# microsoft/tf-gnn-samples

Hardware: AMD Instinct MI355X
Metric: edges/sec (whole node), RGCN PPI h=256 training, distinct batches (the reference's epoch-loop definition) (higher is better)
Workload: dtype f32; 1 GPU; C2: RGCN on synthetic PPI-shaped batches (~16 graphs, ~1.88 M edges, ~32 k nodes each), 3 edge types [fwd,self,bkwd], h=256, 3 layers, sum aggregation, 1/in-de…; graphs_per_rank=64, max_nodes_in_batch=35964, input_pipeline=ResidentDataset, parallelism=dp1-by-graph

## Files before the change

include/relgnn.h:

```cpp
#ifndef RELGNN_H_
#define RELGNN_H_

#include <stddef.h>
#include <stdint.h>

#ifdef __cplusplus
extern "C" {
#endif

#define RELGNN_ABI_VERSION 1

#define RELGNN_OK 0
#define RELGNN_EINVAL 1
#define RELGNN_ENOSPC 2
#define RELGNN_EHIP 3
#define RELGNN_EUNSUPPORTED 4

#define RELGNN_ERRFLAG_INDEX_OUT_OF_RANGE 1u

#define RELGNN_AGG_SUM 0
#define RELGNN_AGG_MEAN 1
#define RELGNN_AGG_SQRT_N 2
#define RELGNN_AGG_MAX 3

// ... 273 lines not shown
                                int32_t batch, uint16_t* out, void* stream);
int relgnn_limb_split_multi_f32(int32_t n, const float* const* X, const int64_t* ldx, const int32_t* rows, const int32_t* cols,
                                const int32_t* transpose, uint16_t* const* out, const int32_t* kt_offset, const int32_t* kt_total,
                                void* stream);
int relgnn_limb_gemm_f32(int32_t act, const uint16_t* A, const uint16_t* B, const float* bias, const void* zeros, float* C,
                         int64_t ldc, int32_t M, int32_t N, int32_t K, void* stream);
int relgnn_limb_gemm_xf32(int32_t act, const float* A, int64_t lda, const uint16_t* B, const float* bias, const void* zeros,
                          float* C, int64_t ldc, int32_t M, int32_t N, int32_t K, void* stream);
int64_t relgnn_limb16_elements(int64_t rows, int64_t cols);
int relgnn_limb16_split_multi_f32(int32_t n, const float* const* X, const int64_t* ldx, const int32_t* rows, const int32_t* cols,
                                  const int32_t* transpose, uint16_t* const* out, const int32_t* kt_offset, const int32_t* kt_total,
                                  const int32_t* image, int32_t n_images, float* wmax, void* stream);
int relgnn_limb16_gemm_xf32(int32_t act, const float* A, int64_t lda, const float* xmax, int32_t xgroups, const uint16_t* B,
                            const float* wmax, const float* bias, const void* zeros, float* C, int64_t ldc, int32_t M, int32_t N,
                            int32_t K, void* stream);
int relgnn_limb16_gemm_tn_f32(const float* A, int64_t lda, const float* G, int64_t ldg, const float* amax, int32_t a_cols_per_scale,
                              const float* gmax, int32_t g_cols_per_scale, float* P, int32_t V, int32_t J, int32_t C, void* stream);
int64_t relgnn_col_absmax_workspace_bytes(int32_t rows, int32_t cols);
int relgnn_col_absmax_f32(const float* X, int64_t ldx, int32_t rows, int32_t cols, float* out, void* workspace,
                          int64_t workspace_bytes, void* stream);
int relgnn_absmax_f32(const float* x, int64_t n, float* out, void* stream);
int relgnn_limb_gemm_xf32_dact(int32_t act, const float* A, int64_t lda, const uint16_t* B, const float* bias, const void* zeros,
                               int32_t dact, const float* Y, int64_t ldy, float* C, int64_t ldc, int32_t M, int32_t N, int32_t K,
                               void* stream);
int relgnn_limb16_gemm_xf32_dact(int32_t act, const float* A, int64_t lda, const float* xmax, int32_t xgroups, const uint16_t* B,
                                 const float* wmax, const float* bias, const void* zeros, int32_t dact, const float* Y, int64_t ldy,
                                 float* C, int64_t ldc, int32_t M, int32_t N, int32_t K, void* stream);
#define RELGNN_HANDOVER_FUSED_MATRIX 1
#define RELGNN_HANDOVER_FUSED_GATHER 2
#define RELGNN_HANDOVER_PC_MATRIX 4
#define RELGNN_HANDOVER_PC_PRODUCER 8
int relgnn_limb_gemm_xf32_pc(int32_t act, const float* A, int64_t lda, const uint16_t* B, const float* bias, int32_t dact,
                             const float* Y, int64_t ldy, float* C, int64_t ldc, int32_t M, int32_t N, int32_t K, int32_t* status,
                             void* stream);
int relgnn_limb_gemm_xf32_pc_supported(int32_t act, int32_t M, int32_t N, int32_t K);
int relgnn_rgcn_fused_fwd(const float* H, int64_t num_rows_h, int64_t ldh, const int32_t* rowptr, int32_t num_nodes,
                          int32_t num_edge_types, const int32_t* col, const float* w, const uint16_t* w_limbs, const float* bias,
                          int32_t act, float* bucket_sums, int64_t lds, float* out, int64_t ldo, int32_t d_in, int32_t d_out,
                          int32_t* status, void* stream);
int relgnn_limb_dense_sel_f32(int32_t layout, int32_t act, const float* A, int64_t lda, const int32_t* a_rows, const float* B,
                              int64_t ldb, int32_t num_b, int64_t b_batch_stride, const int32_t* b_select, int32_t rows_per_select,
                              const float* bias, const void* zeros, uint16_t* limb_ws, int64_t limb_ws_elements, float* C,
                              int64_t ldc, int32_t M, int32_t N, int32_t K, void* stream);
int relgnn_limb_gemm_sel_xf32(int32_t act, const float* A, int64_t lda, const int32_t* a_rows, const uint16_t* B_limbs, int32_t num_b,
                              const int32_t* b_select, int32_t rows_per_select, const float* bias, const void* zeros, float* C,
                              int64_t ldc, int32_t M, int32_t N, int32_t K, void* stream);
int relgnn_limb_gemm_sel_pc_supported(int32_t M, int32_t N, int32_t K, int32_t rows_per_select);
int relgnn_limb_gemm_sel_pc_xf32(const float* A, int64_t lda, const int32_t* a_rows, const uint16_t* B_limbs, int32_t num_b,
                                 const int32_t* b_select, int32_t rows_per_select, const void* zeros, float* C, int64_t ldc,
                                 int32_t M, int32_t N, int32_t K, int32_t* status, void* stream);
int64_t relgnn_limb_gemm_tn_chunks(int32_t V, int32_t J, int32_t C);
int relgnn_limb_gemm_tn_f32(const float* A, int64_t lda, const float* G, int64_t ldg, float* P, int32_t V, int32_t J, int32_t C,
                            void* stream);
int relgnn_limb_gemm_tn_tiles_f32(const float* A, int64_t lda, const int32_t* a_rows, const float* G, int64_t ldg,
                                  const void* zeros, float* part, int32_t P, int32_t rows_per_tile, int32_t J, int32_t C,
                                  void* stream);
int relgnn_limb_dense_f32(int32_t layout, int32_t act, const float* A, int64_t lda, const float* B, int64_t ldb, const float* bias,
                          const void* zeros, uint16_t* limb_ws, int64_t limb_ws_elements, float* C, int64_t ldc, int32_t M,
                          int32_t N, int32_t K, void* stream);


int relgnn_rgdcn_apply_fwd(int32_t mode, int32_t weight_act, int32_t out_act, const float* A, const float* P,
                           int64_t p_node_stride, int64_t p_type_stride, int64_t p_channel_stride, int32_t num_nodes,
                           int32_t num_edge_types, int32_t num_channels, int32_t channel_dim, const int32_t* rowptr_t,
                           float* out, void* stream);
int relgnn_rgdcn_apply_bwd(int32_t weight_act, const float* A, const float* P, int64_t p_node_stride, int64_t p_type_stride,
                           int64_t p_channel_stride, int32_t num_nodes, int32_t num_edge_types, int32_t num_channels,
                           int32_t channel_dim, const float* G, float* gA, float* gP, void* stream);

#ifdef __cplusplus
}
#endif
#endif
```

tf_gnn_samples_amd/_lib.py:

```python
import ctypes
from pathlib import Path

import torch

_PKG_DIR = Path(__file__).resolve().parent
LIB_PATH = _PKG_DIR / "librelgnn.so"

OK, EINVAL, ENOSPC, EHIP, EUNSUPPORTED = 0, 1, 2, 3, 4
ERRFLAG_INDEX_OUT_OF_RANGE = 1

AGG_SUM, AGG_MEAN, AGG_SQRT_N, AGG_MAX = 0, 1, 2, 3
MT_MAX = 48
ACT_LINEAR, ACT_TANH, ACT_RELU, ACT_LEAKY_RELU, ACT_ELU, ACT_SELU, ACT_GELU = range(7)
ACT_NAMES = ("linear", "tanh", "relu", "leaky_relu", "elu", "selu", "gelu")

_c_i32, _c_i64, _c_f32 = ctypes.c_int32, ctypes.c_int64, ctypes.c_float
_ptr = ctypes.c_void_p

_SIGNATURES = {
    "relgnn_abi_version": (ctypes.c_int, []),
    "relgnn_status_string": (ctypes.c_char_p, [ctypes.c_int]),
    "relgnn_relational_keys": (ctypes.c_int, [_ptr, _c_i64, _c_i32, _c_i32, _c_i32, _c_i64, _ptr, _ptr, _ptr, _ptr]),
    "relgnn_relational_keys2": (ctypes.c_int, [_ptr, _c_i64, _c_i32, _c_i32, _c_i32, _c_i64, _ptr, _ptr, _ptr, _ptr, _ptr, _ptr]),
    "relgnn_relational_keys_all": (ctypes.c_int, [_ptr, _ptr, _c_i32, _c_i32, _ptr, _ptr, _ptr, _ptr, _ptr, _ptr]),
# ... 23 lines not shown
    "relgnn_rgat_bwd_logits": (ctypes.c_int, [_ptr, _c_i64, _c_i32, _c_i32, _ptr, _ptr, _ptr, _c_i32, _c_i32, _ptr, _c_f32, _ptr, _ptr, _ptr, _c_i64, _ptr, _ptr, _ptr]),
    "relgnn_rgat_bwd_msg": (ctypes.c_int, [_c_i32, _c_i32, _ptr, _c_i64, _ptr, _ptr, _ptr, _ptr, _ptr, _c_i64, _ptr, _c_i64, _ptr, _ptr]),
    "relgnn_rgat_alpha": (ctypes.c_int, [_ptr, _ptr, _c_i32, _ptr, _c_i32, _c_i32, _ptr, _c_f32, _ptr, _ptr]),
    "relgnn_headw_reduce": (ctypes.c_int, [_ptr, _c_i64, _c_i64, _c_i32, _c_i32, _ptr, _c_i64, _c_i32, _ptr, _ptr, _ptr, _ptr, _c_i64, _ptr, _ptr, _ptr]),
    "relgnn_rgat_dz": (ctypes.c_int, [_ptr, _c_i64, _c_i64, _c_i32, _c_i32, _ptr, _ptr, _ptr, _c_i32, _c_i32, _ptr, _c_f32, _ptr, _ptr, _ptr, _c_i64, _ptr, _ptr, _ptr]),
    "relgnn_pair_fwd": (ctypes.c_int, [_c_i32, _c_i32, _ptr, _c_i64, _ptr, _c_i64, _c_i32, _ptr, _c_i32, _c_i32, _ptr, _ptr, _ptr, _c_i64, _ptr]),
    "relgnn_pair_bwd_q": (ctypes.c_int, [_c_i32, _ptr, _c_i64, _ptr, _c_i64, _c_i32, _ptr, _c_i32, _c_i32, _ptr, _ptr, _ptr, _c_i64, _ptr, _c_i64, _ptr, _ptr]),
    "relgnn_pair_bwd_p": (ctypes.c_int, [_c_i32, _ptr, _c_i64, _ptr, _c_i64, _c_i32, _ptr, _c_i64, _ptr, _ptr, _ptr, _ptr, _c_i64, _ptr, _c_i64, _ptr]),
    "relgnn_column_sum_workspace_bytes": (ctypes.c_size_t, [_c_i64, _c_i32]),
    "relgnn_column_sum": (ctypes.c_int, [_ptr, _c_i64, _c_i32, _c_i64, _ptr, _ptr, ctypes.c_size_t, _ptr]),
    "relgnn_mt_l2norm_workspace_bytes": (ctypes.c_size_t, []),
    "relgnn_mt_l2norm": (ctypes.c_int, [_ptr, _ptr, _c_i32, _ptr, _ptr, ctypes.c_size_t, _ptr]),
    "relgnn_mt_adam_clip": (ctypes.c_int, [_ptr, _ptr, _ptr, _ptr, _ptr, _c_i32, _ptr, _c_f32, _c_f32, _c_f32, _c_f32, _c_f32, _ptr]),
    "relgnn_adam_step_size": (ctypes.c_int, [_ptr, _c_f32, _c_f32, _c_f32, _ptr]),
    "relgnn_mt_adam_clip_devlr": (ctypes.c_int, [_ptr, _ptr, _ptr, _ptr, _ptr, _c_i32, _ptr, _c_f32, _ptr, _c_f32, _c_f32, _c_f32, _ptr]),
    "relgnn_sigmoid_ce_stats_workspace_bytes": (ctypes.c_size_t, []),
    "relgnn_sigmoid_ce_stats": (ctypes.c_int, [_ptr, _ptr, _c_i64, _c_f32, _ptr, _ptr, ctypes.c_size_t, _ptr]),
    "relgnn_sigmoid_ce_bwd": (ctypes.c_int, [_ptr, _ptr, _c_i64, _ptr, _c_f32, _ptr, _ptr, _ptr]),
    "relgnn_sigmoid_ce_bwd_padded": (ctypes.c_int, [_ptr, _ptr, _c_i64, _c_i32, _ptr, _c_f32, _ptr, _ptr, _c_i32, _ptr]),
    "relgnn_gru_gates_fwd": (ctypes.c_int, [_ptr, _ptr, _ptr, _c_i64, _c_i32, _ptr, _ptr, _ptr, _ptr]),
    "relgnn_gru_cell_fwd_supported": (ctypes.c_int, [_c_i32, _c_i32, _c_i32]),
    "relgnn_gru_cell_fwd_xf32": (ctypes.c_int, [_ptr, _c_i64, _ptr, _c_i64, _ptr, _ptr, _ptr, _c_i32, _ptr, _ptr, _ptr, _ptr, _ptr,
                                                _c_i64, _c_i32, _c_i32, _ptr, _ptr]),
    "relgnn_gru_cell_bwd_xf32": (ctypes.c_int, [_ptr, _c_i64, _ptr, _ptr, _ptr, _c_i64, _ptr, _ptr, _ptr, _c_i32, _ptr, _ptr, _ptr, _c_i64,
                                                _c_i32, _c_i32, _ptr, _ptr]),
    "relgnn_gru_out_fwd": (ctypes.c_int, [_ptr, _ptr, _ptr, _ptr, _c_i64, _c_i32, _c_i32, _ptr, _ptr, _ptr]),
    "relgnn_gru_out_bwd": (ctypes.c_int, [_ptr, _ptr, _ptr, _ptr, _c_i64, _c_i32, _c_i32, _ptr, _ptr, _ptr, _ptr, _ptr]),
    "relgnn_gru_gates_bwd": (ctypes.c_int, [_ptr, _ptr, _ptr, _ptr, _ptr, _c_i64, _c_i32, _ptr, _ptr, _ptr]),
    "relgnn_pair_materialize": (ctypes.c_int, [_c_i32, _ptr, _c_i64, _ptr, _c_i64, _c_i32, _ptr, _ptr, _c_i64, _ptr, _ptr, _c_i64, _ptr]),
    "relgnn_rgat_scores_groups": (_c_i64, [_c_i64]),
    "relgnn_rgat_scores_fwd": (ctypes.c_int, [_ptr, _c_i64, _c_i32, _c_i32, _ptr, _c_i32, _c_i64, _ptr, _ptr, _ptr]),
    "relgnn_rgat_scores_bwd": (ctypes.c_int, [_ptr, _c_i64, _c_i32, _c_i32, _ptr, _c_i32, _c_i64, _ptr, _ptr, _ptr, _c_i64, _ptr, _c_i64, _ptr]),
    "relgnn_layer_norm_groups": (_c_i64, [_c_i64, _c_i32]),
    "relgnn_layer_norm_fwd": (ctypes.c_int, [_ptr, _c_i64, _c_i64, _c_i32, _ptr, _ptr, _c_f32, _ptr, _c_i64, _ptr, _ptr, _ptr]),
    "relgnn_layer_norm_bwd": (ctypes.c_int, [_ptr, _c_i64, _ptr, _c_i64, _c_i64, _c_i32, _ptr, _ptr, _ptr, _ptr, _c_i64, _ptr, _c_i64, _ptr]),
    "relgnn_panel_gemm_zeros_floats": (ctypes.c_int, []),
    "relgnn_panel_gemm_f32": (ctypes.c_int, [_c_i32, _c_i32, _ptr, _c_i64, _ptr, _ptr, _c_i64, _ptr, _c_i32, _c_i64, _ptr, _ptr, _ptr,
                                             _c_i64, _c_i32, _c_i32, _c_i32, _c_i32, _c_i64, _c_i64, _c_i64, _c_i32, _ptr]),
    "relgnn_limb_elements": (_c_i64, [_c_i64, _c_i64]),
    "relgnn_limb_split_f32": (ctypes.c_int, [_ptr, _c_i64, _c_i32, _c_i32, _c_i32, _ptr, _ptr]),
    "relgnn_limb_gemm_f32": (ctypes.c_int, [_c_i32, _ptr, _ptr, _ptr, _ptr, _ptr, _c_i64, _c_i32, _c_i32, _c_i32, _ptr]),
    "relgnn_limb_gemm_xf32": (ctypes.c_int, [_c_i32, _ptr, _c_i64, _ptr, _ptr, _ptr, _ptr, _c_i64, _c_i32, _c_i32, _c_i32, _ptr]),
    "relgnn_limb_gemm_xf32_dact": (ctypes.c_int, [_c_i32, _ptr, _c_i64, _ptr, _ptr, _ptr, _c_i32, _ptr, _c_i64, _ptr, _c_i64, _c_i32, _c_i32,
                                                  _c_i32, _ptr]),
    "relgnn_limb16_gemm_xf32_dact": (ctypes.c_int, [_c_i32, _ptr, _c_i64, _ptr, _c_i32, _ptr, _ptr, _ptr, _ptr, _c_i32, _ptr, _c_i64, _ptr,
                                                    _c_i64, _c_i32, _c_i32, _c_i32, _ptr]),
    "relgnn_rgcn_fused_fwd": (ctypes.c_int, [_ptr, _c_i64, _c_i64, _ptr, _c_i32, _c_i32, _ptr, _ptr, _ptr, _ptr, _c_i32, _ptr, _c_i64, _ptr,
                                             _c_i64, _c_i32, _c_i32, _ptr, _ptr]),
    "relgnn_limb_gemm_xf32_pc": (ctypes.c_int, [_c_i32, _ptr, _c_i64, _ptr, _ptr, _c_i32, _ptr, _c_i64, _ptr, _c_i64, _c_i32, _c_i32, _c_i32,
                                                _ptr, _ptr]),
    "relgnn_limb_gemm_xf32_pc_supported": (ctypes.c_int, [_c_i32, _c_i32, _c_i32, _c_i32]),
    "relgnn_limb_gemm_tn_chunks": (_c_i64, [_c_i32, _c_i32, _c_i32]),
    "relgnn_limb_gemm_tn_f32": (ctypes.c_int, [_ptr, _c_i64, _ptr, _c_i64, _ptr, _c_i32, _c_i32, _c_i32, _ptr]),
    "relgnn_limb_gemm_tn_tiles_f32": (ctypes.c_int, [_ptr, _c_i64, _ptr, _ptr, _c_i64, _ptr, _ptr, _c_i32, _c_i32, _c_i32, _c_i32, _ptr]),
    "relgnn_limb16_gemm_tn_f32": (ctypes.c_int, [_ptr, _c_i64, _ptr, _c_i64, _ptr, _c_i32, _ptr, _c_i32, _ptr, _c_i32, _c_i32, _c_i32, _ptr]),
    "relgnn_col_absmax_workspace_bytes": (ctypes.c_int64, [_c_i32, _c_i32]),
    "relgnn_col_absmax_f32": (ctypes.c_int, [_ptr, _c_i64, _c_i32, _c_i32, _ptr, _ptr, _c_i64, _ptr]),
    "relgnn_absmax_f32": (ctypes.c_int, [_ptr, _c_i64, _ptr, _ptr]),
    "relgnn_limb16_elements": (_c_i64, [_c_i64, _c_i64]),
    "relgnn_limb16_split_multi_f32": (ctypes.c_int, [_c_i32, _ptr, _ptr, _ptr, _ptr, _ptr, _ptr, _ptr, _ptr, _ptr, _c_i32, _ptr, _ptr]),
    "relgnn_limb16_gemm_xf32": (ctypes.c_int, [_c_i32, _ptr, _c_i64, _ptr, _c_i32, _ptr, _ptr, _ptr, _ptr, _ptr, _c_i64, _c_i32, _c_i32,
                                               _c_i32, _ptr]),
    "relgnn_limb_split_multi_f32": (ctypes.c_int, [_c_i32, _ptr, _ptr, _ptr, _ptr, _ptr, _ptr, _ptr, _ptr, _ptr]),
    "relgnn_limb_split_batch_f32": (ctypes.c_int, [_ptr, _c_i64, _c_i64, _c_i32, _c_i32, _c_i32, _c_i32, _ptr, _ptr]),
    "relgnn_limb_dense_sel_f32": (ctypes.c_int, [_c_i32, _c_i32, _ptr, _c_i64, _ptr, _ptr, _c_i64, _c_i32, _c_i64, _ptr, _c_i32, _ptr, _ptr,
                                                 _ptr, _c_i64, _ptr, _c_i64, _c_i32, _c_i32, _c_i32, _ptr]),
    "relgnn_limb_gemm_sel_xf32": (ctypes.c_int, [_c_i32, _ptr, _c_i64, _ptr, _ptr, _c_i32, _ptr, _c_i32, _ptr, _ptr, _ptr, _c_i64, _c_i32,
                                                 _c_i32, _c_i32, _ptr]),
    "relgnn_limb_gemm_sel_pc_supported": (ctypes.c_int, [_c_i32, _c_i32, _c_i32, _c_i32]),
    "relgnn_limb_gemm_sel_pc_xf32": (ctypes.c_int, [_ptr, _c_i64, _ptr, _ptr, _c_i32, _ptr, _c_i32, _ptr, _ptr, _c_i64, _c_i32, _c_i32,
                                                    _c_i32, _ptr, _ptr]),
    "relgnn_fill_rows_f32": (ctypes.c_int, [_ptr, _c_i64, _c_i32, _ptr, _c_i64, ctypes.c_float, _ptr]),
    "relgnn_limb_dense_f32": (ctypes.c_int, [_c_i32, _c_i32, _ptr, _c_i64, _ptr, _c_i64, _ptr, _ptr, _ptr, _c_i64, _ptr, _c_i64, _c_i32,
                                             _c_i32, _c_i32, _ptr]),
    "relgnn_blaslt_gemm_f32": (ctypes.c_int, [_c_i32, _c_i32, _ptr, _c_i64, _ptr, _c_i64, _ptr, _ptr, _c_i64, _c_i32, _c_i32, _c_i32, _c_i32,
                                              _c_i64, _c_i64, _c_i64, _c_i32, _ptr, _c_i64, _ptr]),
    "relgnn_gemm_tn_stream_workspace_bytes": (_c_i64, [_c_i32, _c_i32, _c_i64]),
    "relgnn_gemm_tn_stream_f32": (ctypes.c_int, [_ptr, _c_i64, _ptr, _c_i64, _ptr, _c_i64, _c_i32, _c_i32, _c_i64, _c_i32, _ptr, _c_i64, _ptr]),
    "relgnn_gemm_tn_stream_group_workspace_bytes": (_c_i64, [_c_i32, _ptr, _ptr, _c_i64, _c_i32]),
    "relgnn_gemm_tn_stream_group_f32": (ctypes.c_int, [_c_i32, _ptr, _ptr, _ptr, _ptr, _ptr, _ptr, _ptr, _ptr, _c_i64, _ptr, _ptr, _c_i64,
                                                       _ptr]),
    "relgnn_gemm_tn_stream_blocks_f32": (ctypes.c_int, [_ptr, _c_i64, _ptr, _c_i64, _ptr, _c_i64, _c_i64, _c_i32, _c_i32, _c_i32, _c_i64,
                                                        _c_i32, _ptr, _c_i64, _ptr]),
    "relgnn_sum_slabs_tail_f32": (ctypes.c_int, [_ptr, _c_i32, _c_i32, _c_i32, _ptr, _c_i64, _ptr, _c_i64, _c_i32, _ptr, _ptr]),
    "relgnn_rgdcn_apply_fwd": (ctypes.c_int, [_c_i32, _c_i32, _c_i32, _ptr, _ptr, _c_i64, _c_i64, _c_i64, _c_i32, _c_i32, _c_i32, _c_i32, _ptr, _ptr, _ptr]),
    "relgnn_rgdcn_apply_bwd": (ctypes.c_int, [_c_i32, _ptr, _ptr, _c_i64, _c_i64, _c_i64, _c_i32, _c_i32, _c_i32, _c_i32, _ptr, _ptr, _ptr, _ptr]),
    "relgnn_batch_gather": (ctypes.c_int, [_ptr, _c_i32, _c_i32, _c_i64] + [_ptr] * 6 + [_c_i64, _c_i64, _c_i64, _c_i32, _ptr, _ptr, _ptr,
                                           _ptr, _ptr, _ptr, _ptr, _ptr, _ptr]),
    "relgnn_plan_assemble": (ctypes.c_int, [_ptr, _c_i32, _c_i32, _c_i64] + [_ptr] * 8 + [_c_i64, _c_i64] + [_ptr] * 16 + [_ptr] * 5 + [_ptr]),
    "relgnn_batch_layout_len": (_c_i64, [_c_i32, _c_i32]),
    "relgnn_batch_count": (_c_i64, [_ptr, _ptr, _c_i64, _c_i64, _c_i64]),
    "relgnn_batch_layout": (ctypes.c_int, [_c_i32, _c_i64, _ptr, _ptr, _ptr, _c_i32, _ptr, _ptr]),
    "relgnn_batch_pack": (ctypes.c_int, [_c_i32, _c_i64, _ptr, _ptr, _ptr, _ptr, _ptr, _c_i32, _ptr, _ptr, _ptr, _ptr, ctypes.c_size_t, _c_i32]),
}

_lib = None


class RelGnnLibraryError(RuntimeError):
    pass


def load_library():
    global _lib
    if _lib is not None:
        return _lib
# ... 53 lines not shown
```

tf_gnn_samples_amd/csrc/limb_gemm.hip:

```cpp
#include "common.h"
#include "lds_dma.h"
#include "limb_split.h"

#include <stdlib.h>
#include <type_traits>

using namespace relgnn;

namespace {

typedef float f32x4 __attribute__((ext_vector_type(4)));
typedef float f32x16 __attribute__((ext_vector_type(16)));
typedef __bf16 bf16x8 __attribute__((ext_vector_type(8)));
constexpr int BK = 16;
constexpr int STAGES = 4;
#ifdef RELGNN_LIMB_TIMING
__device__ unsigned long long* g_limb_timing_dev = nullptr;
unsigned long long* g_limb_timing = nullptr;
#define TSTAMP(v) __builtin_amdgcn_sched_barrier(0); const unsigned long long v = __builtin_amdgcn_s_memtime(); __builtin_amdgcn_sched_barrier(0)
#else
#define TSTAMP(v)
#endif

struct LimbArgs {
// ... 712 lines not shown
      TSTAMP(q1);
      x_load(xv[j], ptr_nxt, j);
      const Limbs wb = read_w(2 * j + 1), xb0 = read_x(2 * j + 1, 0), xb1 = read_x(2 * j + 1, 1);
      two(wa, xa0, xa1);
      two(wb, xb0, xb1);
      TSTAMP(q2);
      if constexpr (j == 3) store_panel(p);
      TSTAMP(q3);
      wait_lgkm0();
      TSTAMP(q4);
      __builtin_amdgcn_s_barrier();
      __builtin_amdgcn_sched_barrier(0);
#ifdef RELGNN_LIMB_TIMING
      { TSTAMP(q5); seg[1] += q1 - q0; seg[2] += q2 - q1; seg[3] += q3 - q2; seg[4] += q4 - q3; seg[5] += q5 - q4; }
#endif
    };
    supertile(std::integral_constant<int, 0>{});
    supertile(std::integral_constant<int, 1>{});
    supertile(std::integral_constant<int, 2>{});
    supertile(std::integral_constant<int, 3>{});
    ok_cur = ok_nxt;
    id_nxt = id_nn;
    id_nn = id_n3;
    if (p + 1 < np) {
      const int t = type_of(p + 1);
      if (t != type_cur) {
        type_cur = t;
        load_w(t);
        wait_vm<0>();
        __builtin_amdgcn_s_barrier();
        __builtin_amdgcn_sched_barrier(0);
      }
    }
  }
#ifdef RELGNN_LIMB_TIMING
  if (g_limb_timing_dev && lane == 0 && lb < 64) {
    TSTAMP(t_end);
    seg[6] = t_end - t_begin; seg[7] = np;
#pragma unroll
    for (int i = 0; i < 8; ++i) g_limb_timing_dev[(lb * 8 + wave) * 8 + i] = seg[i];
  }
#endif
}

struct LimbTnArgs {
  const float* A; int64_t lda;
  const float* G; int64_t ldg;
  float* P;
  int32_t V, J, C;
  int32_t rows_per_chunk;
  int32_t panels, chunks, Z;
  const float* amax; const float* gmax; int32_t a_cols, g_cols;
  const int32_t* a_rows; const float* zeros;
};

template <int T32, int NL = 3, int NC = 256, bool GATHER = false>
__global__ __launch_bounds__(512) void limb_gemm_tn_kernel(const LimbTnArgs a) {
  constexpr int PR = 32 * T32;
  constexpr int CW = NC / 32, RW = 8 / CW, TPW = T32 / RW;
  static_assert((NC == 256 || NC == 128) && T32 % RW == 0 && TPW >= 1, "wave roles");
  constexpr int PA = NL * T32, PB = NL * (NC / 32), P = PA + PB;
  constexpr int STAGE_BYTES = P * 1024;
  constexpr int XG = PR / 4;
  constexpr int GG = NC / 4;
  constexpr int ITEMS = NC + 4 * XG;
  static_assert(ITEMS <= 512 && STAGES * STAGE_BYTES <= 160 * 1024, "geometry");
  constexpr int DUMP = STAGES * STAGE_BYTES;
  __shared__ __attribute__((aligned(16))) unsigned char lds[STAGES * STAGE_BYTES + 3072];

  const int tid = threadIdx.x, lane = tid & 63;
  const int wave = __builtin_amdgcn_readfirstlane(tid >> 6);
  const int per_z = a.panels * a.chunks;
  const int64_t lb = xcd_logical_block((int64_t)per_z * a.Z);
  if (lb < 0) return;
  const int z = (int)(lb / per_z), pc = (int)(lb % per_z);
  const int q = pc / a.chunks, chunk = pc % a.chunks;
  const int j0 = q * PR, n0 = chunk * NC;
  const int r_beg = z * a.rows_per_chunk;
  const int r_end = min(a.V, r_beg + a.rows_per_chunk);
  const int ntiles = (r_end - r_beg) / BK;

  const bool is_g = tid < NC;
  const bool active = tid < ITEMS;
  const int idx = is_g ? tid : (active ? tid - NC : 0);
  const int grp = is_g ? (idx % GG) : (idx % XG);
  const int oct = is_g ? (idx / GG) : (idx / XG);
  const int col = 4 * grp;
  const float* base = is_g ? a.G + n0 + col : a.A + j0 + col;
  const int64_t ld = is_g ? a.ldg : a.lda;
  const int blk = ((is_g ? PA : 0) + NL * (col >> 5)) * 1024 + (oct & 1) * 512 + (col & 31) * 16;
  float pscale[4] = {1.f, 1.f, 1.f, 1.f};
  if constexpr (NL == 2) {
#pragma unroll
    for (int c = 0; c < 4; ++c)
      pscale[c] = limb16_scale(is_g ? a.gmax[(n0 + col + c) / a.g_cols] : a.amax[(j0 + col + c) / a.a_cols]);
  }
  const int cswz = ((col & 31) >> 3) & 3;
  const int dump = DUMP + lane * 16;
  f32x4 pv[8];
  float ph[16];
  const int nsuper = ntiles / 2;
  int nix[8] = {0, 0, 0, 0, 0, 0, 0, 0};
  auto ix_load = [&](int S) {
    if constexpr (GATHER) {
      const int r0 = min(r_beg + 32 * S + 8 * oct, a.V - 8);
      const int4 i0 = *reinterpret_cast<const int4*>(a.a_rows + r0), i1 = *reinterpret_cast<const int4*>(a.a_rows + r0 + 4);
      nix[0] = i0.x; nix[1] = i0.y; nix[2] = i0.z; nix[3] = i0.w; nix[4] = i1.x; nix[5] = i1.y; nix[6] = i1.z; nix[7] = i1.w;
    }
  };
  auto p_load = [&](int S) {
    const int r0 = r_beg + 32 * S + 8 * oct;
    if constexpr (GATHER) {
      const float* zsrc = a.zeros;
#pragma unroll
      for (int m = 0; m < 8; ++m) {
        const int64_t row = is_g ? (int64_t)min(r0 + m, a.V - 1) : (int64_t)nix[m];
        const float* p = row >= 0 ? base + row * ld : zsrc;
        pv[m] = *reinterpret_cast<const f32x4*>(p);
      }
      ix_load(S + 1);
    } else {
#pragma unroll
      for (int m = 0; m < 8; ++m) pv[m] = *reinterpret_cast<const f32x4*>(base + (int64_t)min(r0 + m, a.V - 1) * ld);
    }
  };
  auto p_store = [&](int S, int c, const float* v) {
    const int off = (active && S < nsuper) ? ((2 * S + (oct >> 1)) % STAGES) * STAGE_BYTES + blk + (c ^ cswz) * 16 : dump;
// ... 103 lines not shown
          __builtin_amdgcn_s_barrier();
          __builtin_amdgcn_sched_barrier(0);
          w_nxt = read_w((t + 1) % STAGES);
          xn = read_x((t + 1) % STAGES, 0);
        }
      } else {
        xn = read_x(stage, tm + 1);
      }
      acc[tm] = products(acc[tm], w_cur, xc);
      if constexpr (PRE >= 1) {
        if (tm < PRE) {
          constexpr int A_AT = 0, B_AT = PRE >= 2 ? 1 : 0, L_AT = PRE >= 3 ? 2 : PRE - 1;
          if (tm == A_AT) { if constexpr (ODD == 0) p_step(S, I0{}); else p_step(S, I2{}); }
          if (tm == B_AT) { if constexpr (ODD == 0) p_step(S, I1{}); else p_step(S, I3{}); }
          if (tm == L_AT) { if constexpr (ODD == 0) p_load(S + 1); }
          __builtin_amdgcn_sched_barrier(0);
        }
      }
    }
    w_cur = w_nxt;
  };
  {
    int t = 0;
    for (; t + 1 < ntiles; t += 2) {
      ktile(t, I0{});
      ktile(t + 1, I1{});
    }
  }

  const int i32 = lane & 31, h32 = lane >> 5;
  const int colw = n0 + cw * 32;
  float* slab = a.P + (int64_t)z * a.J * a.C;
  int ug[4][4];
  if constexpr (NL == 2) {
#pragma unroll
    for (int c = 0; c < 4; ++c)
#pragma unroll
      for (int e = 0; e < 4; ++e) ug[c][e] = limb16_unscale_exp(a.gmax[(colw + 8 * c + 4 * h32 + e) / a.g_cols]);
  }
#pragma unroll
  for (int tm = 0; tm < TPW; ++tm) {
    const int j = j0 + (tm0 + tm) * 32 + i32;
    float* crow = slab + (int64_t)j * a.C;
    int ua = 0;
    if constexpr (NL == 2) ua = limb16_unscale_exp(a.amax[j / a.a_cols]);
#pragma unroll
    for (int c = 0; c < 4; ++c) {
      f32x4 v = f32x4{acc[tm][4 * c], acc[tm][4 * c + 1], acc[tm][4 * c + 2], acc[tm][4 * c + 3]};
      if constexpr (NL == 2)
        v = f32x4{ldexpf(v[0], ua + ug[c][0]), ldexpf(v[1], ua + ug[c][1]), ldexpf(v[2], ua + ug[c][2]), ldexpf(v[3], ua + ug[c][3])};
      *reinterpret_cast<f32x4*>(crow + colw + 8 * c + 4 * h32) = v;
    }
  }
}

__device__ __forceinline__ uint32_t finite_mag_bits(float x) {
  const uint32_t u = __float_as_uint(x) & 0x7FFFFFFFu;
  return u < 0x7F800000u ? u : 0u;
}
__device__ __forceinline__ float finite_mag(float x) { return __uint_as_float(finite_mag_bits(x)); }

__global__ __launch_bounds__(256) void absmax_kernel(const float* __restrict__ x, int64_t n4, int64_t n, float* __restrict__ out) {
  float m = 0.f;
  const f32x4* x4 = reinterpret_cast<const f32x4*>(x);
  for (int64_t i = (int64_t)blockIdx.x * 256 + threadIdx.x; i < n4; i += (int64_t)gridDim.x * 256) {
    const f32x4 v = x4[i];
    m = fmaxf(fmaxf(m, fmaxf(finite_mag(v[0]), finite_mag(v[1]))), fmaxf(finite_mag(v[2]), finite_mag(v[3])));
  }
  if (blockIdx.x == 0 && threadIdx.x < (n - 4 * n4)) m = fmaxf(m, finite_mag(x[4 * n4 + threadIdx.x]));
#pragma unroll
  for (int o = 32; o > 0; o >>= 1) m = fmaxf(m, __shfl_xor(m, o, 64));
  __shared__ float wave_max[4];
  if ((threadIdx.x & 63) == 0) wave_max[threadIdx.x >> 6] = m;
  __syncthreads();
  if (threadIdx.x == 0) {
    m = fmaxf(fmaxf(wave_max[0], wave_max[1]), fmaxf(wave_max[2], wave_max[3]));
    if (m > 0.f) atomicMax(reinterpret_cast<unsigned int*>(out), __float_as_uint(m));
  }
}

__global__ __launch_bounds__(256) void col_absmax_part_kernel(const float* __restrict__ X, int64_t ldx, int32_t rows, int32_t cols,
                                                              int32_t rows_per_block, uint32_t* __restrict__ part) {
  const int q = blockIdx.x * 64 + (threadIdx.x & 63);
  const int y = threadIdx.x >> 6;
  const int r0 = blockIdx.y * rows_per_block, r1 = min(rows, r0 + rows_per_block);
  uint32_t m[4] = {0u, 0u, 0u, 0u};
  if (4 * q < cols) {
    const float* p = X + 4 * q;
    int r = r0 + y;
    for (; r + 12 < r1; r += 16) {
      f32x4 v[4];
#pragma unroll
      for (int u = 0; u < 4; ++u) v[u] = __builtin_nontemporal_load(reinterpret_cast<const f32x4*>(p + (int64_t)(r + 4 * u) * ldx));
#pragma unroll
      for (int u = 0; u < 4; ++u)
#pragma unroll
        for (int e = 0; e < 4; ++e) m[e] = max(m[e], finite_mag_bits(v[u][e]));
    }
    for (; r < r1; r += 4) {
      const f32x4 v = *reinterpret_cast<const f32x4*>(p + (int64_t)r * ldx);
#pragma unroll
      for (int e = 0; e < 4; ++e) m[e] = max(m[e], finite_mag_bits(v[e]));
    }
  }
  __shared__ uint32_t sh[4][64][4];
#pragma unroll
// ... 495 lines not shown
  dim3 grid((unsigned)gx, (unsigned)nb);
  col_absmax_part_kernel<<<grid, 256, 0, st>>>(X, ldx, rows, cols, per, static_cast<uint32_t*>(workspace));
  int rc = launch_status();
  if (rc != RELGNN_OK) return rc;
  col_absmax_final_kernel<<<(unsigned)((cols + 3) / 4), 256, 0, st>>>(static_cast<const uint32_t*>(workspace), nb, cols, out);
  return launch_status();
}

int relgnn_absmax_f32(const float* x, int64_t n, float* out, void* stream) {
  if (n < 0 || !out) return RELGNN_EINVAL;
  hipStream_t st = as_stream(stream);
  if (hipMemsetAsync(out, 0, sizeof(float), st) != hipSuccess) return RELGNN_EHIP;
  if (n == 0) return RELGNN_OK;
  if (!x) return RELGNN_EINVAL;
  if (!aligned16(x)) return RELGNN_EUNSUPPORTED;
  const int64_t n4 = n / 4;
  int64_t blocks = (n4 + 255) / 256;
  if (blocks > 2048) blocks = 2048;
  if (blocks < 1) blocks = 1;
  absmax_kernel<<<(unsigned)blocks, 256, 0, st>>>(x, n4, n, out);
  return launch_status();
}

static int limb_tn_any(const float* A, int64_t lda, const float* G, int64_t ldg, const float* amax, const float* gmax,
                       int32_t a_cols, int32_t g_cols, float* P, int32_t V, int32_t J, int32_t C, void* stream) {
  if (V < 0 || J < 0 || C < 0) return RELGNN_EINVAL;
  if (J == 0 || C == 0) return RELGNN_OK;
  if (V < 32) return RELGNN_EUNSUPPORTED;
  if (!A || !G || !P) return RELGNN_EINVAL;
  if (J % 32 != 0 || C % 256 != 0 || lda % 4 || ldg % 4 || lda < J || ldg < C || !aligned16(A) || !aligned16(G) || !aligned16(P))
    return RELGNN_EUNSUPPORTED;
  LimbTnArgs a{};
  a.A = A; a.lda = lda; a.G = G; a.ldg = ldg; a.P = P; a.V = V - V % 32; a.J = J; a.C = C; a.amax = amax; a.gmax = gmax;
  a.a_cols = a_cols; a.g_cols = g_cols;
  int t32, rows, Z;
  limb_tn_geometry(V, J, C, &t32, &rows, &Z);
  a.panels = (J / 32) / t32; a.chunks = C / 256; a.rows_per_chunk = rows; a.Z = Z;
  const int64_t logical = (int64_t)a.panels * a.chunks * a.Z;
  const unsigned grid = (unsigned)(8 * ((logical + 7) / 8));
  hipStream_t st = as_stream(stream);
  if (amax) {
    switch (t32) {
      case 4: limb_gemm_tn_kernel<4, 2><<<grid, 512, 0, st>>>(a); break;
      case 2: limb_gemm_tn_kernel<2, 2><<<grid, 512, 0, st>>>(a); break;
      default: limb_gemm_tn_kernel<1, 2><<<grid, 512, 0, st>>>(a); break;
    }
    return launch_status();
  }
  switch (t32) {
    case 4: limb_gemm_tn_kernel<4><<<grid, 512, 0, st>>>(a); break;
    case 2: limb_gemm_tn_kernel<2><<<grid, 512, 0, st>>>(a); break;
    default: limb_gemm_tn_kernel<1><<<grid, 512, 0, st>>>(a); break;
  }
  return launch_status();
}

int relgnn_limb_gemm_tn_tiles_f32(const float* A, int64_t lda, const int32_t* a_rows, const float* G, int64_t ldg,
                                  const void* zeros, float* part, int32_t P, int32_t rows_per_tile, int32_t J, int32_t C,
                                  void* stream) {
  if (P < 0 || J < 0 || C < 0 || rows_per_tile <= 0) return RELGNN_EINVAL;
  if (P == 0 || J == 0 || C == 0) return RELGNN_OK;
  if (!A || !a_rows || !G || !zeros || !part) return RELGNN_EINVAL;
  if (rows_per_tile % 32 != 0 || P % rows_per_tile != 0 || J % 64 != 0 || C % 128 != 0 || lda % 4 || ldg % 4 || lda < J || ldg < C ||
      !aligned16(A) || !aligned16(G) || !aligned16(part) || !aligned16(a_rows) || !aligned16(zeros))
    return RELGNN_EUNSUPPORTED;
  LimbTnArgs a{};
  a.A = A; a.lda = lda; a.G = G; a.ldg = ldg; a.P = part; a.V = P; a.J = J; a.C = C; a.a_cols = 1; a.g_cols = 1;
  a.a_rows = a_rows; a.zeros = static_cast<const float*>(zeros);
  const bool wide = C % 256 == 0;
  const int t32 = J % 128 == 0 ? 4 : 2;
  a.panels = (J / 32) / t32; a.chunks = C / (wide ? 256 : 128); a.rows_per_chunk = rows_per_tile; a.Z = P / rows_per_tile;
  const int64_t logical = (int64_t)a.panels * a.chunks * a.Z;
  const unsigned grid = (unsigned)(8 * ((logical + 7) / 8));
  hipStream_t st = as_stream(stream);
  if (wide) {
    if (t32 == 4) limb_gemm_tn_kernel<4, 3, 256, true><<<grid, 512, 0, st>>>(a);
    else limb_gemm_tn_kernel<2, 3, 256, true><<<grid, 512, 0, st>>>(a);
  } else {
    if (t32 == 4) limb_gemm_tn_kernel<4, 3, 128, true><<<grid, 512, 0, st>>>(a);
    else limb_gemm_tn_kernel<2, 3, 128, true><<<grid, 512, 0, st>>>(a);
  }
  return launch_status();
}

static int limb_sel_launch(int32_t act, const float* A, int64_t lda, const int32_t* a_rows, const uint16_t* limbs, int64_t per,
                           const int32_t* b_select, int32_t rows_per_select, const float* bias, const void* zeros, float* C,
                           int64_t ldc, int32_t M, int32_t N, int32_t n_valid, int32_t K, bool cut, void* stream) {
  LimbSelArgs a{};
  a.n_valid = n_valid;
  a.Ax = A; a.lda = lda; a.rows = a_rows; a.B = limbs; a.b_select = b_select; a.rows_per_select = rows_per_select; a.b_stride = per;
  a.bias = bias; a.zeros = static_cast<const uint16_t*>(zeros); a.C = C; a.ldc = ldc; a.M = M; a.N = N; a.K = K; a.act = act;
  a.chunks = N / 128;
  static const bool tile_form = []() { const char* e = getenv("RELGNN_LIMB_TILE"); return !(e && e[0] == '0'); }();
  if (tile_form && !cut && K == 128 && M >= 128 * 256 && (b_select || (int64_t)M * a.chunks >= (int64_t)128 * 256 * 4)) {
    if (!b_select) a.rows_per_select = 128;
    a.panels = 256 / a.chunks > 0 ? 256 / a.chunks : 1;
    const int64_t logical = (int64_t)a.panels * a.chunks;
    limb_gemm_tile_kernel<<<(unsigned)(8 * ((logical + 7) / 8)), 512, 0, as_stream(stream)>>>(a);
    return launch_status();
  }
  a.panels = (M + 127) / 128;
  const int64_t logical = (int64_t)a.panels * a.chunks;
  limb_gemm_sel_kernel<<<(unsigned)(8 * ((logical + 7) / 8)), 512, 0, as_stream(stream)>>>(a);
  return launch_status();
}

// ... 57 lines not shown
```

tf_gnn_samples_amd/dense.py:

```python
import os

import torch

from .config import settings as _cfg



def _ops():
    from . import ops
    return ops


_LIMB_MIN_ROWS, _LIMB_MAX_K = 4096, 1024
GEMM_NN, GEMM_NT, GEMM_TN = 0, 1, 2
_WARNED_UNSUPPORTED = False


_FROM_OUTPUT_ACTS = (1, 2, 3, 4, 5)
_IDEMPOTENT_ACTS = (2,)


def mark_activation_output(y: torch.Tensor, act: int, sole_consumer: bool = False) -> torch.Tensor:
    if act in _FROM_OUTPUT_ACTS and y.is_cuda and y.dtype == torch.float32 and y.dim() == 2:
        y._relgnn_act = (int(act), y._version, bool(sole_consumer))
# ... 730 lines not shown
            and a_rows.data_ptr() % 16 == 0 and a_rows.numel() == g.shape[0] and rows_per_tile % 32 == 0
            and g.shape[0] % rows_per_tile == 0 and a.shape[1] % 64 == 0 and g.shape[1] % 128 == 0)


def limb_gemm_tn_tiles(a: torch.Tensor, g: torch.Tensor, a_rows: torch.Tensor, rows_per_tile: int) -> torch.Tensor:
    from . import _lib
    lib = _lib.load_library()
    P, C = g.shape
    J = a.shape[1]
    tiles = P // rows_per_tile
    part = torch.empty((tiles, J, C), dtype=torch.float32, device=g.device)
    _lib.check(lib.relgnn_limb_gemm_tn_tiles_f32(a.data_ptr(), a.stride(0), a_rows.data_ptr(), g.data_ptr(), g.stride(0),
                                                 _lib.ptr(_zeros(g.device)), part.data_ptr(), P, int(rows_per_tile), J, C,
                                                 _lib.current_stream()), "relgnn_limb_gemm_tn_tiles_f32")
    return part


def col_absmax(x: torch.Tensor) -> torch.Tensor:
    from . import _lib
    lib = _lib.load_library()
    cols = x.shape[1]
    if cols > 16 and cols % 4:
        return col_absmax(torch.nn.functional.pad(x, (0, (-cols) % 4)))[:cols]
    if x.shape[1] > 16 and not _rows_ok(x):
        x = x.contiguous()
    if x.shape[1] <= 16 and not (x.is_cuda and x.dtype == torch.float32 and x.dim() == 2 and x.stride(1) == 1):
        x = x.contiguous()
    out = torch.empty(x.shape[1], dtype=torch.float32, device=x.device)
    nbytes = int(lib.relgnn_col_absmax_workspace_bytes(x.shape[0], x.shape[1]))
    ws = torch.empty(nbytes // 4, dtype=torch.int32, device=x.device) if nbytes else None
    _lib.check(lib.relgnn_col_absmax_f32(_lib.ptr(x, rows_strided=True), x.stride(0) if x.shape[0] > 1 else x.shape[1], x.shape[0],
                                         x.shape[1], out.data_ptr(), _lib.ptr(ws), nbytes, _lib.current_stream()),
               "relgnn_col_absmax_f32")
    return out


def absmax(x: torch.Tensor) -> torch.Tensor:
    from . import _lib
    x = x if x.is_contiguous() else x.contiguous()
    out = torch.empty(1, dtype=torch.float32, device=x.device)
    _lib.check(_lib.load_library().relgnn_absmax_f32(_lib.ptr(x), x.numel(), out.data_ptr(), _lib.current_stream()), "relgnn_absmax_f32")
    return out


def limb_gemm_tn(a: torch.Tensor, b: torch.Tensor, amax: torch.Tensor = None, bmax: torch.Tensor = None) -> torch.Tensor:
    from . import _lib
    lib = _lib.load_library()
    V, J = a.shape
    C = b.shape[1]
    Z = int(lib.relgnn_limb_gemm_tn_chunks(V, J, C))
    if Z <= 0:
        raise ValueError("limb_gemm_tn: unsupported shape [%d, %d]^T @ [%d, %d]" % (V, J, V, C))
    parts = torch.empty((Z, J, C), dtype=torch.float32, device=a.device)
    if amax is not None:
        na, nb = amax.numel(), bmax.numel()
        if na < 1 or nb < 1 or J % na or C % nb or amax.dtype != torch.float32 or bmax.dtype != torch.float32:
            raise ValueError("limb_gemm_tn: the magnitude counts (%d, %d) must divide the operand widths (%d, %d)" % (na, nb, J, C))
        _lib.check(lib.relgnn_limb16_gemm_tn_f32(a.data_ptr(), a.stride(0), b.data_ptr(), b.stride(0), amax.data_ptr(), J // na,
                                                 bmax.data_ptr(), C // nb, parts.data_ptr(), V, J, C, _lib.current_stream()),
                   "relgnn_limb16_gemm_tn_f32")
    else:
        _lib.check(lib.relgnn_limb_gemm_tn_f32(a.data_ptr(), a.stride(0), b.data_ptr(), b.stride(0), parts.data_ptr(), V, J, C,
                                               _lib.current_stream()), "relgnn_limb_gemm_tn_f32")
    R = V % 32
    out = torch.empty((J, C), dtype=torch.float32, device=a.device)
    _lib.check(lib.relgnn_sum_slabs_tail_f32(_lib.ptr(parts), Z, J, C, a[V - R:].data_ptr() if R else None, a.stride(0),
                                             b[V - R:].data_ptr() if R else None, b.stride(0), R, _lib.ptr(out),
                                             _lib.current_stream()), "relgnn_sum_slabs_tail_f32")
    return out


def enable_gemm_autotuning(max_tuning_ms_per_solution: int = 30, tune: bool = True) -> bool:
    import os
    import tempfile
    tun = getattr(torch.cuda, "tunable", None)
    if tun is None or not torch.cuda.is_available():
        return False
    try:
        tun.enable(True)
        tun.tuning_enable(bool(tune))
    except Exception:
        return False
    for fn, arg in (("set_filename", os.path.join(tempfile.gettempdir(), "relgnn_tunableop_%d.csv" % os.getpid())),
                    ("set_max_tuning_duration", int(max_tuning_ms_per_solution))):
        try:
            if tune:
                getattr(tun, fn)(arg)
        except Exception:
            pass
    return True


def _split_count(V: int, M: int, N: int) -> int:
    tiles = max(1, ((M + 127) // 128) * ((N + 127) // 128))
    want = max(1, 512 // tiles)
    return int(max(1, min(want, V // 512, 64)))


def tn_stream_into(a: torch.Tensor, b: torch.Tensor, out: torch.Tensor) -> None:
    from . import _lib
    lib = _lib.load_library()
    V, M = a.shape
    N = b.shape[1]
    if out.shape != (M, N) or out.stride(1) != 1 or out.dtype != torch.float32:
        raise ValueError("tn_stream_into: out must be a float32 [%d, %d] block with dense rows" % (M, N))
    nbytes = lib.relgnn_gemm_tn_stream_workspace_bytes(M, N, V)
# ... 257 lines not shown
```

Measured before the change: 1.068 billion edges/sec.

## Fuse split-K slab reduction into limb TN GEMM via last-arriver tile sum

Adds a TN GEMM variant where each split-K block writes its partial slab, then increments a per-tile arrival counter, and the last arriving block sums all Z partials plus the V%32 tail rows and writes the final output. This removes the separate sum_slabs_tail kernel launch and its extra pass over the partials. The new kernel uses 256-thread, 4-wave blocks with 128-wide column chunks instead of 512 threads and 256-wide chunks, which changes occupancy and tiling. In exchange it needs a zeroed counter buffer per call and makes the final reduction serial in whichever block arrives last.

```diff
diff --git a/include/relgnn.h b/include/relgnn.h
--- a/include/relgnn.h
+++ b/include/relgnn.h
@@ -349,6 +349,8 @@
 int64_t relgnn_limb_gemm_tn_chunks(int32_t V, int32_t J, int32_t C);
 int relgnn_limb_gemm_tn_f32(const float* A, int64_t lda, const float* G, int64_t ldg, float* P, int32_t V, int32_t J, int32_t C,
                             void* stream);
+int relgnn_limb_gemm_tn_sum_f32(const float* A, int64_t lda, const float* G, int64_t ldg, float* P, uint32_t* arrivals, float* out,
+                                int32_t V, int32_t J, int32_t C, void* stream);
 int relgnn_limb_gemm_tn_tiles_f32(const float* A, int64_t lda, const int32_t* a_rows, const float* G, int64_t ldg,
                                   const void* zeros, float* part, int32_t P, int32_t rows_per_tile, int32_t J, int32_t C,
                                   void* stream);
diff --git a/tf_gnn_samples_amd/_lib.py b/tf_gnn_samples_amd/_lib.py
--- a/tf_gnn_samples_amd/_lib.py
+++ b/tf_gnn_samples_amd/_lib.py
@@ -99,6 +99,7 @@
     "relgnn_limb_gemm_xf32_pc_supported": (ctypes.c_int, [_c_i32, _c_i32, _c_i32, _c_i32]),
     "relgnn_limb_gemm_tn_chunks": (_c_i64, [_c_i32, _c_i32, _c_i32]),
     "relgnn_limb_gemm_tn_f32": (ctypes.c_int, [_ptr, _c_i64, _ptr, _c_i64, _ptr, _c_i32, _c_i32, _c_i32, _ptr]),
+    "relgnn_limb_gemm_tn_sum_f32": (ctypes.c_int, [_ptr, _c_i64, _ptr, _c_i64, _ptr, _ptr, _ptr, _c_i32, _c_i32, _c_i32, _ptr]),
     "relgnn_limb_gemm_tn_tiles_f32": (ctypes.c_int, [_ptr, _c_i64, _ptr, _ptr, _c_i64, _ptr, _ptr, _c_i32, _c_i32, _c_i32, _c_i32, _ptr]),
     "relgnn_limb16_gemm_tn_f32": (ctypes.c_int, [_ptr, _c_i64, _ptr, _c_i64, _ptr, _c_i32, _ptr, _c_i32, _ptr, _c_i32, _c_i32, _c_i32, _ptr]),
     "relgnn_col_absmax_workspace_bytes": (ctypes.c_int64, [_c_i32, _c_i32]),
diff --git a/tf_gnn_samples_amd/csrc/limb_gemm.hip b/tf_gnn_samples_amd/csrc/limb_gemm.hip
--- a/tf_gnn_samples_amd/csrc/limb_gemm.hip
+++ b/tf_gnn_samples_amd/csrc/limb_gemm.hip
@@ -788,19 +788,20 @@
   int32_t panels, chunks, Z;
   const float* amax; const float* gmax; int32_t a_cols, g_cols;
   const int32_t* a_rows; const float* zeros;
+  unsigned* arrivals; float* out; const float* At; const float* Gt; int32_t R;
 };
 
-template <int T32, int NL = 3, int NC = 256, bool GATHER = false>
-__global__ __launch_bounds__(512) void limb_gemm_tn_kernel(const LimbTnArgs a) {
+template <int T32, int NL, int NC, bool GATHER, int NW>
+__device__ __forceinline__ int limb_tn_partial(const LimbTnArgs& a) {
   constexpr int PR = 32 * T32;
-  constexpr int CW = NC / 32, RW = 8 / CW, TPW = T32 / RW;
-  static_assert((NC == 256 || NC == 128) && T32 % RW == 0 && TPW >= 1, "wave roles");
+  constexpr int CW = NC / 32, RW = NW / CW, TPW = T32 / RW;
+  static_assert((NC == 256 || NC == 128) && (NW == 8 || NW == 4) && RW >= 1 && T32 % RW == 0 && TPW >= 1, "wave roles");
   constexpr int PA = NL * T32, PB = NL * (NC / 32), P = PA + PB;
   constexpr int STAGE_BYTES = P * 1024;
   constexpr int XG = PR / 4;
   constexpr int GG = NC / 4;
   constexpr int ITEMS = NC + 4 * XG;
-  static_assert(ITEMS <= 512 && STAGES * STAGE_BYTES <= 160 * 1024, "geometry");
+  static_assert(ITEMS <= 64 * NW && STAGES * STAGE_BYTES <= 160 * 1024, "geometry");
   constexpr int DUMP = STAGES * STAGE_BYTES;
   __shared__ __attribute__((aligned(16))) unsigned char lds[STAGES * STAGE_BYTES + 3072];
 
@@ -808,7 +809,7 @@
   const int wave = __builtin_amdgcn_readfirstlane(tid >> 6);
   const int per_z = a.panels * a.chunks;
   const int64_t lb = xcd_logical_block((int64_t)per_z * a.Z);
-  if (lb < 0) return;
+  if (lb < 0) return -1;
   const int z = (int)(lb / per_z), pc = (int)(lb % per_z);
   const int q = pc / a.chunks, chunk = pc % a.chunks;
   const int j0 = q * PR, n0 = chunk * NC;
@@ -1018,6 +1019,68 @@
       *reinterpret_cast<f32x4*>(crow + colw + 8 * c + 4 * h32) = v;
     }
   }
+  return pc;
+}
+
+template <int T32, int NL = 3, int NC = 256, bool GATHER = false>
+__global__ __launch_bounds__(512) void limb_gemm_tn_kernel(const LimbTnArgs a) {
+  limb_tn_partial<T32, NL, NC, GATHER, 8>(a);
+}
+
+template <int T32>
+__global__ __launch_bounds__(256, 2) void limb_gemm_tn_sum_kernel(const LimbTnArgs a) {
+  constexpr int NC = 128, PR = 32 * T32;
+  const int tile = limb_tn_partial<T32, 3, NC, false, 4>(a);
+  if (tile < 0) return;
+  __shared__ int last;
+  __threadfence();
+  __syncthreads();
+  if (threadIdx.x == 0) last = atomicAdd(a.arrivals + tile, 1u) == (unsigned)(a.Z - 1);
+  __syncthreads();
+  if (!last) return;
+  __threadfence();
+  const int q = tile / a.chunks, chunk = tile % a.chunks;
+  const int j0 = q * PR, n0 = chunk * NC;
+  const int64_t jc = (int64_t)a.J * a.C;
+  constexpr int G4 = NC / 4, GROUPS = PR * G4, U = 4;
+  static_assert(GROUPS % (256 * U) == 0, "sum passes");
+  const int tid = threadIdx.x;
+#pragma unroll 1
+  for (int p = 0; p < GROUPS; p += 256 * U) {
+    int row[U], col[U];
+    int64_t off[U];
+    f32x4 s0[U], s1[U];
+#pragma unroll
+    for (int u = 0; u < U; ++u) {
+      const int e = p + u * 256 + tid;
+      row[u] = j0 + e / G4; col[u] = n0 + 4 * (e % G4);
+      off[u] = (int64_t)row[u] * a.C + col[u];
+      s0[u] = f32x4{0.f, 0.f, 0.f, 0.f}; s1[u] = s0[u];
+    }
+    int z = 0;
+    for (; z + 1 < a.Z; z += 2) {
+      const float* p0 = a.P + (int64_t)z * jc;
+#pragma unroll
+      for (int u = 0; u < U; ++u) {
+        s0[u] += *reinterpret_cast<const f32x4*>(p0 + off[u]);
+        s1[u] += *reinterpret_cast<const f32x4*>(p0 + jc + off[u]);
+      }
+    }
+    if (z < a.Z) {
+#pragma unroll
+      for (int u = 0; u < U; ++u) s0[u] += *reinterpret_cast<const f32x4*>(a.P + (int64_t)z * jc + off[u]);
+    }
+#pragma unroll
+    for (int u = 0; u < U; ++u) {
+      f32x4 s = s0[u] + s1[u];
+      for (int r = 0; r < a.R; ++r) {
+        const float x = a.At[(int64_t)r * a.lda + row[u]];
+        const f32x4 g = *reinterpret_cast<const f32x4*>(a.Gt + (int64_t)r * a.ldg + col[u]);
+        s = f32x4{fmaf(x, g[0], s[0]), fmaf(x, g[1], s[1]), fmaf(x, g[2], s[2]), fmaf(x, g[3], s[3])};
+      }
+      *reinterpret_cast<f32x4*>(a.out + off[u]) = s;
+    }
+  }
 }
 
 __device__ __forceinline__ uint32_t finite_mag_bits(float x) {
@@ -1619,6 +1682,27 @@
     case 2: limb_gemm_tn_kernel<2><<<grid, 512, 0, st>>>(a); break;
     default: limb_gemm_tn_kernel<1><<<grid, 512, 0, st>>>(a); break;
   }
+  return launch_status();
+}
+
+int relgnn_limb_gemm_tn_sum_f32(const float* A, int64_t lda, const float* G, int64_t ldg, float* P, uint32_t* arrivals, float* out,
+                                int32_t V, int32_t J, int32_t C, void* stream) {
+  if (V < 0 || J < 0 || C < 0) return RELGNN_EINVAL;
+  if (J == 0 || C == 0) return RELGNN_OK;
+  if (V < 32) return RELGNN_EUNSUPPORTED;
+  if (!A || !G || !P || !arrivals || !out) return RELGNN_EINVAL;
+  if (J % 128 != 0 || C % 256 != 0 || lda % 4 || ldg % 4 || lda < J || ldg < C || !aligned16(A) || !aligned16(G) || !aligned16(P) ||
+      !aligned16(out))
+    return RELGNN_EUNSUPPORTED;
+  LimbTnArgs a{};
+  const int32_t R = V % 32;
+  a.A = A; a.lda = lda; a.G = G; a.ldg = ldg; a.P = P; a.V = V - R; a.J = J; a.C = C; a.a_cols = 1; a.g_cols = 1;
+  a.arrivals = arrivals; a.out = out; a.At = A + (int64_t)(V - R) * lda; a.Gt = G + (int64_t)(V - R) * ldg; a.R = R;
+  int t32, rows, Z;
+  limb_tn_geometry(V, J, C, &t32, &rows, &Z);
+  a.panels = J / 128; a.chunks = C / 128; a.rows_per_chunk = rows; a.Z = Z;
+  const int64_t logical = (int64_t)a.panels * a.chunks * a.Z;
+  limb_gemm_tn_sum_kernel<4><<<(unsigned)(8 * ((logical + 7) / 8)), 256, 0, as_stream(stream)>>>(a);
   return launch_status();
 }
 
diff --git a/tf_gnn_samples_amd/dense.py b/tf_gnn_samples_amd/dense.py
--- a/tf_gnn_samples_amd/dense.py
+++ b/tf_gnn_samples_amd/dense.py
@@ -806,6 +806,13 @@
     if Z <= 0:
         raise ValueError("limb_gemm_tn: unsupported shape [%d, %d]^T @ [%d, %d]" % (V, J, V, C))
     parts = torch.empty((Z, J, C), dtype=torch.float32, device=a.device)
+    if amax is None and J % 128 == 0:
+        out = torch.empty((J, C), dtype=torch.float32, device=a.device)
+        arrivals = torch.zeros((J // 128) * (C // 128), dtype=torch.int32, device=a.device)
+        _lib.check(lib.relgnn_limb_gemm_tn_sum_f32(a.data_ptr(), a.stride(0), b.data_ptr(), b.stride(0), parts.data_ptr(),
+                                                   arrivals.data_ptr(), out.data_ptr(), V, J, C, _lib.current_stream()),
+                   "relgnn_limb_gemm_tn_sum_f32")
+        return out
     if amax is not None:
         na, nb = amax.numel(), bmax.numel()
         if na < 1 or nb < 1 or J % na or C % nb or amax.dtype != torch.float32 or bmax.dtype != torch.float32:
```

New measurement: 859.1 million edges/sec (median of 2 runs). 19.6% lower.
